# shincling/DL4SS

Measured on AMD Instinct MI355X. Metric: mixtures/sec (8 kHz, 4 s, 2-spk WSJ0-shape) at 1/2/4/8 MI355X, higher is better.
Workload: dtype bf16; 1 GPU; C2: 2-spk pit BiLSTM-4L magnitude mask (EvalVer model), B=32/GPU, N=32000 (T=251,F=129); global_batch=32, seq_len=251, parallelism=dp1, precision=bf16, loss=pit, launch=hip-graph, step=mix+STFT+fwd+loss+bwd+allreduce+Adam

## Files before the change

### dl4ss_amd/csrc/gemm_gl.hip

```cpp
#include "common.h"

#include <algorithm>

namespace {

typedef short bf16x8 __attribute__((ext_vector_type(8)));
typedef short bf16x4 __attribute__((ext_vector_type(4)));
typedef float f32x4 __attribute__((ext_vector_type(4)));
typedef __attribute__((address_space(3))) void lds_void;
typedef __attribute__((address_space(3))) bf16x4 lds_bf16x4;

constexpr int BN = 128, BK = 64;
constexpr int PAN = 128 * BK;

template <int BM_, int STG_, int KT_ = 64>
struct Cfg {
  static constexpr int BM = BM_, STG = STG_, KT = KT_, NT = 2 * BM_, NW = NT / 64;
  static constexpr int PPP = KT_ / 4;
  static constexpr int CPW_A = BM_ * KT_ / 512 / NW, CPW_B = BN * KT_ / 512 / NW;
  static constexpr int IMG_A = BM_ * KT_, IMG_B = BN * KT_, STAGE = IMG_A + IMG_B;
  static constexpr int SMEM = STG_ * STAGE > NW * 32 * 68 * 2 ? STG_ * STAGE : NW * 32 * 68 * 2;
  static constexpr int WPC = NT > 256 ? 1 : SMEM * 2 <= 40 * 1024 ? 4 : SMEM * 2 <= 53 * 1024 ? 3
                             : SMEM * 2 <= 80 * 1024 ? 2 : 1;
  static_assert(CPW_A >= 1 && CPW_B >= 1, "at least one DMA per wave and operand");
// ... 117 lines not shown
#pragma unroll
    for (int kk = 0; kk < KT / 32; ++kk) {
      bf16x8 af[4], bfr[4];
#pragma unroll
      for (int i = 0; i < 4; ++i) af[i] = frag<A_KC, KT>(ia, wm + 16 * i + (lane & 15), kk, lane);
#pragma unroll
      for (int j = 0; j < 4; ++j) bfr[j] = frag<B_KC, KT>(ib, wn + 16 * j + (lane & 15), kk, lane);
#ifndef GGL_NO_MFMA
#pragma unroll
      for (int i = 0; i < 4; ++i)
#pragma unroll
        for (int j = 0; j < 4; ++j) acc[i][j] = __builtin_amdgcn_mfma_f32_16x16x32_bf16(af[i], bfr[j], acc[i][j], 0, 0, 0);
      if constexpr (RS) {
        if (rs) {
#pragma unroll
          for (int i = 0; i < 4; ++i) accr[i] = __builtin_amdgcn_mfma_f32_16x16x32_bf16(af[i], ones, accr[i], 0, 0, 0);
        }
      }
#else
#pragma unroll
      for (int i = 0; i < 4; ++i) asm volatile("" :: "v"(af[i]), "v"(bfr[i]));
#endif
    }
  };
  auto dma = [&](int t) {
    unsigned short* na = smem + (t % STG) * STAGE;
    sa_.issue(na, wave, t, t * KT, kspan);
    sb_.issue(na + IMG_A, wave, t, t * KT, kspan);
  };
  if constexpr (STG == 2) {
    dma(0);
    asm volatile("s_waitcnt vmcnt(0)" ::: "memory");
    __syncthreads();
    for (int kt = 0; kt < nk; ++kt) {
#ifndef GGL_NO_DMA
      if (kt + 1 < nk) dma(kt + 1);
#endif
      compute(smem + (kt & 1) * STAGE);
      asm volatile("s_waitcnt vmcnt(0)" ::: "memory");
      __syncthreads();
    }
  } else {
    constexpr int PW = CF::CPW_A + CF::CPW_B;
#pragma unroll
    for (int t = 0; t < STG - 1; ++t)
      if (t < nk) dma(t);
    for (int kt = 0; kt < nk; ++kt) {
      const int ahead = min(STG - 2, nk - 1 - kt);
      if (ahead >= STG - 2) vm_wait<(STG - 2) * PW>();
      else vm_wait_n<PW, STG - 2>(ahead);
      __builtin_amdgcn_s_barrier();
      if (kt + STG - 1 < nk) dma(kt + STG - 1);
      compute(smem + (kt % STG) * STAGE);
    }
    __syncthreads();
  }

  if constexpr (RS) {
    if (rs && (lane & 15) == 0) {
#pragma unroll
      for (int i = 0; i < 4; ++i)
#pragma unroll
        for (int e = 0; e < 4; ++e) {
          const int row = m0 + wm + 16 * i + 4 * (lane >> 4) + e;
          if (row < M) rsum[row] = beta != 0.0f ? accr[i][e] + beta * rsum[row] : accr[i][e];
        }
    }
  }
  constexpr int SLD = 68;
  float* stage = reinterpret_cast<float*>(smem) + wave * 32 * SLD;
  const int c4 = 4 * (lane & 15);
  const int col = n0 + wn + c4;
  const bool add_bias = !SPLIT && bias != nullptr;
  float4 bv = make_float4(0.f, 0.f, 0.f, 0.f);
  if (add_bias) {
    bv.x = col < N ? bias[col] : 0.f;
    bv.y = col + 1 < N ? bias[col + 1] : 0.f;
    bv.z = col + 2 < N ? bias[col + 2] : 0.f;
    bv.w = col + 3 < N ? bias[col + 3] : 0.f;
  }
  float* out = SPLIT ? slab : C;
  const long long ldo = SPLIT ? N : ldc;
  const bool vec_c = (ldo % 4 == 0) && ((((uintptr_t)out) & 15) == 0) && col + 4 <= N;
#pragma unroll
  for (int h = 0; h < 2; ++h) {
#ifdef GGL_NO_STORE
    if (M > 0) break;
#endif
    __builtin_amdgcn_wave_barrier();
    asm volatile("" ::: "memory");
#pragma unroll
    for (int i2 = 0; i2 < 2; ++i2)
#pragma unroll
      for (int j = 0; j < 4; ++j)
#pragma unroll
        for (int e = 0; e < 4; ++e)
          stage[(16 * i2 + 4 * (lane >> 4) + e) * SLD + 16 * j + (lane & 15)] = acc[2 * h + i2][j][e];
    __builtin_amdgcn_wave_barrier();
    asm volatile("" ::: "memory");
#pragma unroll 4
    for (int rr = 0; rr < 32; rr += 4) {
      const int rl = rr + (lane >> 4);
      const int row = m0 + wm + 32 * h + rl;
      if (row >= M) continue;
      float4 x = *reinterpret_cast<const float4*>(stage + rl * SLD + c4);
      x.x += bv.x; x.y += bv.y; x.z += bv.z; x.w += bv.w;
      if constexpr (EPI == EPI_TANH_BF16) {
        unsigned short* cb = reinterpret_cast<unsigned short*>(C) + (long long)row * ldc + col;
        const float xs[4] = {ftanh_fast(x.x), ftanh_fast(x.y), ftanh_fast(x.z), ftanh_fast(x.w)};
        unsigned short hb[4];
#pragma unroll
        for (int c = 0; c < 4; ++c) {
          hb[c] = (unsigned short)bf16_bits_rne(xs[c]);
        }
        if (col + 4 <= N) {
          *reinterpret_cast<unsigned*>(cb) = hb[0] | ((unsigned)hb[1] << 16);
          *reinterpret_cast<unsigned*>(cb + 2) = hb[2] | ((unsigned)hb[3] << 16);
        } else {
          for (int c = 0; c < 4 && col + c < N; ++c) cb[c] = hb[c];
        }
        continue;
      }
      float* cp = out + (long long)row * ldo + col;
      if (vec_c) {
        if (!SPLIT && beta != 0.0f) {
          const float4 o = *reinterpret_cast<const float4*>(cp);
          x.x += beta * o.x; x.y += beta * o.y; x.z += beta * o.z; x.w += beta * o.w;
        }
        if (EPI == EPI_TANH) { x.x = ftanh_fast(x.x); x.y = ftanh_fast(x.y); x.z = ftanh_fast(x.z); x.w = ftanh_fast(x.w); }
        *reinterpret_cast<float4*>(cp) = x;
      } else {
        const float xs[4] = {x.x, x.y, x.z, x.w};
#pragma unroll
        for (int c = 0; c < 4; ++c) {
          if (col + c >= N) break;
          float y = xs[c];
          if (!SPLIT && beta != 0.0f) y += beta * cp[c];
          if (EPI == EPI_TANH) y = ftanh_fast(y);
          cp[c] = y;
        }
      }
    }
  }
}

template <bool A_KC, bool B_KC, int EPI, bool SPLIT, class CF>
__global__ __launch_bounds__(CF::NT, CF::WPC) void gemm_gl_kernel(
    int M, int N, int K, const unsigned short* __restrict__ A, long long lda, const unsigned short* __restrict__ B,
    long long ldb, float* __restrict__ C, long long ldc, const float* __restrict__ bias, float beta, int k_per_split,
    int grid_m, int grid_n, long long sa, long long sb, long long sc, float* __restrict__ part) {
  constexpr int BM = CF::BM;
  __shared__ __attribute__((aligned(16))) unsigned short smem[CF::SMEM];
  const int ntiles = grid_m * grid_n;
  const int nwg = gridDim.x * gridDim.y * gridDim.z;
  const int L = blockIdx.x + gridDim.x * (blockIdx.y + gridDim.y * blockIdx.z);
  const int xcd = L % 8, q8 = nwg / 8, r8 = nwg % 8;
  const int R = (xcd < r8 ? xcd * (q8 + 1) : r8 * (q8 + 1) + (xcd - r8) * q8) + L / 8;
  const int zsplit = R / (ntiles * (int)gridDim.y);
  const int ymem = (R / ntiles) % (int)gridDim.y;
  const int tile = R % ntiles;
  A += ymem * sa;
  B += ymem * sb;
  C += ymem * sc;
  constexpr int GROUP = 8;
  const int gsize = GROUP * grid_n;
  const int first_m = (tile / gsize) * GROUP;
  const int gm_here = min(grid_m - first_m, GROUP);
  const int tm = first_m + (tile % gsize) % gm_here, tn = (tile % gsize) / gm_here;
  const int m0 = tm * BM, n0 = tn * BN;
  const int kbeg = zsplit * k_per_split;
  const int kend = min(K, kbeg + k_per_split);
  if (kbeg >= kend) return;
  gl_tile<A_KC, B_KC, EPI, SPLIT, CF>(smem, M, N, A, lda, B, ldb, C, ldc, bias, beta, m0, n0, kbeg, kend - kbeg,
                                      SPLIT ? part + ((long long)ymem * gridDim.z + zsplit) * M * N : nullptr);
}

template <int EPI, bool SPLIT>
__device__ __forceinline__ void store4(float4 x, int row, int col, int N, float* C, long long ldc, float* out,
                                       long long ldo, bool vec_c, float beta, const float4& bv) {
  x.x += bv.x; x.y += bv.y; x.z += bv.z; x.w += bv.w;
  if constexpr (EPI == EPI_TANH_BF16) {
    unsigned short* cb = reinterpret_cast<unsigned short*>(C) + (long long)row * ldc + col;
// ... 632 lines not shown
```

### dl4ss_amd/engine.py

```python
import ctypes

import torch

from . import _lib, adam, dp, ops
from .adversarial import AdvStep
from .ops import CELLS, DEFER_BIAS, DGH_PAD8, DOUT_SLABS, WS_ZEROED, pad8
from .params import DiscNet, FlatParams, SepNet, _ngate
from .plan import RETIRED_KNOBS, check_args, step_plan
from .imagequery import ImageQueryStep
from .voiceprint import VoiceprintStep


class SepTrainer:

    def __init__(self, net, batch, k, n_samples, mode="label", precision="fp32", lr=2e-4, sum_weight=0.5,
                 loss_channels=None, betas=(0.9, 0.999), eps=1e-8, process_group=None, rnn_precision=None,
                 adversary=None, adv_weight=1.0, adv_lr=None, disc_adv_update=True, clip_norm=None,
                 adv_clip_norm=None, voiceprint=None, memory=None, voiceprint_lr=None, memory_refresh="reference",
                 splitk_reduce="atomic", image_query=None, image_query_lr=None, optimizer="adam",
                 schedule_decay=0.004, clipnorm=None):
        self.clip_norm, self.adv_clip_norm = check_args(
            net, batch, k, n_samples, mode, precision, rnn_precision, loss_channels, process_group, adversary,
            clip_norm, adv_clip_norm, voiceprint, memory, memory_refresh, splitk_reduce=splitk_reduce,
            inet=image_query, optimizer=optimizer, schedule_decay=schedule_decay, clipnorm=clipnorm)
        self.optimizer, self.schedule_decay = optimizer, float(schedule_decay)
        self.clipnorm = None if clipnorm is None else float(clipnorm)
        self.inet = image_query
        self.vnet, self.memory, self.memory_refresh, self.adversary = voiceprint, memory, memory_refresh, adversary
        self.align = getattr(net, "attention", "dot") == "align"
        vars(self).update(vars(step_plan(net, batch, n_samples, precision, rnn_precision, process_group)))
        self.net, self.B, self.K, self.N = net, batch, k, n_samples
        self.mode, self.precision = mode, precision
        self._sk = 1 if (self.align and not self.fast) else "auto"
        self.splitk_reduce = splitk_reduce
        self._gk = {}
        if splitk_reduce == "fixed":
            self._sk = "auto"
        self.pg = process_group
        self.world = dp.world(process_group) if process_group is not None else 1
        self.T = ops.n_frames(n_samples)
        self.F = net.F
        dev = net.device
        B, K, N, T, F, H = batch, k, n_samples, self.T, net.F, net.H
        NGH = _ngate(net.cell) * H
        BT, FE = B * T, F * net.E
        f32 = dict(device=dev, dtype=torch.float32)
        self._sig = torch.empty(B + B * K, N, **f32)
        self.mix = self._sig[:B]
        self.src = self._sig[B:].view(B, K, N)
        self.stats = torch.empty(32 * B * K, **f32)
        if mode == "crm":
            self.mag_mix = torch.empty(B, T, F, **f32)
            self.Xc_mix = torch.empty(B, T, F, 2, **f32)
            self.Xc_src = torch.empty(B, K, T, F, 2, **f32)
        else:
            self.Xc_mix = None
            self._mag = torch.empty(B + B * K * (2 if adversary is not None else 1), T, F, **f32)
            self.mag_mix = self._mag[:B]
            self.mag_src = self._mag[B:B + B * K].view(B, K, T, F)
        self.out = [torch.empty(B, T, 2 * H, **f32) for _ in range(net.L)]
        self.hprev = [torch.empty(B, T, 2 * H, **f32) for _ in range(net.L)]
        self.act = [torch.empty(B, T, 2, 4 * H, **f32) for _ in range(net.L)]
        self.cs = [torch.empty(B, T, 2, H, **f32) for _ in range(net.L)] if net.cell == "lstm" else None
        self.G = torch.empty(BT, 2 * NGH, **f32)
        self.dGh = torch.empty(BT, 2 * NGH, **f32) if net.cell == "gru" else None
        self.dH = [torch.empty(BT, 2 * H, **f32), torch.empty(BT, 2 * H, **f32)]
        self.V = torch.empty(BT, FE, **f32)
        if splitk_reduce == "fixed":
            shapes = [(FE, 2 * H, BT), (BT, 2 * H, FE), (NGH, H, BT), (BT, 2 * H, 2 * NGH)]
            shapes += [(2 * NGH, F if l == 0 else 2 * H, BT) for l in range(net.L)]
            nb = max(ops.gemm_fixed_ws_bytes(*s, "auto") for s in shapes)
            self.fixed_ws = torch.empty(max(nb, 4) // 4, **f32)
            self.cs_part = ops.vp_colsum_part(BT, max(FE, 2 * NGH), dev)
            self._gk = dict(reduce="fixed", ws=self.fixed_ws)
        W = net.W
        self.q = torch.empty(B, K, W, **f32)
        self.mean = torch.empty(B, 2 * H, **f32)
        self.dq = torch.empty(B, K, W, **f32)
        self.dh_bcast = torch.empty(B, 2 * H, **f32)
        self.nblk = _lib.query("dl4ss_attn_align_nblk", T * F) if self.align else _lib.query("dl4ss_attn_nblk", T, F)
        self.part_loss = torch.empty(B, self.nblk, K * K + 1, **f32)
        self.part_dq = torch.empty(B, self.nblk, K, W, **f32)
        if self.align:
            self.part_att = torch.empty(_lib.query("dl4ss_attn_align_part_floats", B, K, self.nblk), **f32)
        self.perm = torch.empty(B, K, device=dev, dtype=torch.int32)
        self.loss = torch.zeros(3, **f32)
        self.eval_out = torch.zeros(3, **f32)
        ws = _lib.query("dl4ss_birnn_workspace_bytes", CELLS[net.cell], B, H)
        if ws < 0:
            raise RuntimeError("unsupported BiRNN configuration")
        self.ws_bytes = ws
        self.rnn_ws = torch.empty((ws + 7) // 8, device=dev, dtype=torch.int64)
        w8 = (ws + 255) // 256 * 32
        self.rnn_ws_all = torch.zeros(2, net.L * w8, device=dev, dtype=torch.int64)
        self._w8 = w8
        self.status = torch.zeros(2, device=dev, dtype=torch.int32)
        okw = dict(kind=optimizer, schedule_decay=schedule_decay, clipnorm=self.clipnorm)
        query_net = voiceprint if voiceprint is not None else image_query
        if self.clipnorm is not None and query_net is not None:
            n0 = ops.grad_sumsq_parts(net.flat.numel())
            joint = torch.zeros(n0 + ops.grad_sumsq_parts(query_net.flat.numel()), dtype=torch.float64, device=dev)
            okw.update(parts=(joint, 0))
        self.opt = adam.GuardedAdam(net.flat, self.status, self.loss, lr, betas, eps, clip_norm=self.clip_norm, **okw)
        if okw.get("parts"):
            okw.update(parts=(joint, n0))
        self.m, self.v = self.opt.m, self.opt.v
        if self.opt.clip is not None:
            self.grad_norm, self._nonfinite = self.opt.grad_norm, self.opt.nonfinite
        nch = loss_channels if loss_channels else K
        self.s1 = 1.0 / (B * nch * T * F)
        self.s2 = 0.0 if (mode == "crm" or loss_channels) else sum_weight / (B * T * F)
        self.spk = torch.empty(B, K, device=dev, dtype=torch.int32)
        self._works = []
        self._in_chain = False
        self._side_stream = self._side_gemm = self._fork_ev = None
        self._wb_ver = None
        self.adv = self.adv_opt = self.vp = None
        if adversary is not None:
            self.adv = AdvStep(adversary, B, K, self._mag, precision, self.status, self.loss,
                               lr if adv_lr is None else adv_lr, betas, eps, adv_weight, disc_adv_update,
                               self.adv_clip_norm)
            a = self.adv
            self.adv_opt, self.adv_m, self.adv_v, self.adv_weight = a.opt, a.opt.m, a.opt.v, a.adv_weight
            self.adv_loss, self.adv_scores, self.gext, self._dmaps, self._dy = a.adv_loss, a.scores, a.gext, a.maps, a.y
            if self.adv_clip_norm is not None:
                self.adv_grad_norm = self.adv_opt.grad_norm
        if voiceprint is not None:
            self.vp = VoiceprintStep(voiceprint, memory, memory_refresh, self.mag_src, self.spk, self.q, self.dq,
                                     self.status, self.loss, lr if voiceprint_lr is None else voiceprint_lr, betas, eps,
                                     wgrad_split="auto" if splitk_reduce == "fixed" else 1, opt_kw=okw)
            self.vp_enc, self.vp_opt = self.vp.enc, self.vp.opt
        self.images = None
        if image_query is not None:
            self.images = torch.zeros(B, K, image_query.h, image_query.w, **f32)
            self.vp = ImageQueryStep(image_query, memory, memory_refresh, self.images, self.spk, self.q, self.dq,
                                     self.status, self.loss, lr if image_query_lr is None else image_query_lr, betas,
                                     eps, opt_kw=okw)
            self.vp_enc, self.vp_opt = self.vp.enc, self.vp.opt
        if not self.fast:
            return
        bf = dict(device=dev, dtype=torch.bfloat16)
        self.xb0 = torch.zeros(BT, pad8(F), **bf)
        self.outb = [torch.empty(BT, pad8(2 * H), **bf) for _ in range(net.L)]
        self.hprevb = [torch.empty(BT, 2 * pad8(H), **bf) for _ in range(net.L)]
        self.dGb_l = [torch.empty(BT, 2 * NGH, **bf) for _ in range(net.L)]
        self.ngh_p8 = pad8(NGH)
        self.dGhb_l = [torch.empty(BT, 2 * self.ngh_p8, **bf) for _ in range(net.L)] if net.cell == "gru" else None
        self._dw_group = None
        self.dPreb = torch.zeros(BT, pad8(FE), **bf)
        gl_need = max(_lib.query("dl4ss_gemm_bf16_gl_ws_bytes", BT, 2 * H, FE, max(1, self.dh_split), 1),
                      _lib.query("dl4ss_gemm_bf16_gl_ws_bytes", BT, 2 * H, 2 * NGH, 1, 1),
                      _lib.query("dl4ss_gemm_bf16_gl_ws_bytes", FE, 2 * H, BT, 2, 1),
                      _lib.query("dl4ss_gemm_bf16_gl_ws_bytes", 2 * NGH, 2 * H, BT, 4, 1),
                      _lib.query("dl4ss_gemm_bf16_gl_ws_bytes", NGH, H, BT, 8, 2))
        self.gl_ws = torch.empty(max(gl_need, 1), device=dev, dtype=torch.uint8)
        if self.dh_slabs > 1:
            self.dh_ws = torch.empty(self.dh_slabs * BT * 2 * H * 4, device=dev, dtype=torch.uint8)
        pb = _lib.query("dl4ss_colsum_bf16_part_bytes", BT, FE)
        self.colsum_part = torch.empty(max(1, pb // 4), device=dev, dtype=torch.float32)
        self.Vb = None if self.split else torch.empty(BT, FE, **bf)
        self.wb_ih = [torch.empty(2 * NGH, pad8(F if l == 0 else 2 * H), **bf) for l in range(net.L)]
        self.wb_lin = torch.empty(FE, pad8(2 * H), **bf)
        if self.split:
            self.seg = [pad8(F if l == 0 else 2 * H) for l in range(net.L)]
            self.xs0 = torch.empty(BT, 3 * self.seg[0], **bf)
            self.xs = torch.empty(BT, 3 * pad8(2 * H), **bf)
            self.ws_ih = [torch.empty(2 * NGH, 3 * self.seg[l], **bf) for l in range(net.L)]
            self.ws_lin = torch.empty(FE, 3 * pad8(2 * H), **bf)
        if net.cell == "lstm":
            self.hprev = [None] * net.L

    lr, adv_lr, vp_lr = (adam.delegate(o, "lr") for o in ("opt", "adv_opt", "vp_opt"))
    step_count = adam.delegate("opt", "step_count")
    skipped_nonfinite = adam.delegate("opt", "skipped_nonfinite")
    adv_step_count = adam.delegate("adv_opt", "step_count")
    adv_skipped_nonfinite = adam.delegate("adv_opt", "skipped_nonfinite", default=0)

    def features(self, raw, gains, lengths=None):
        ops.mix_sources(raw, gains, out_src=self.src, out_mix=self.mix, stats_ws=self.stats, lengths=lengths)
        self._stfts()

    def _stfts(self):
        B, K, N = self.B, self.K, self.N
        xb = dict(out_bf16=self.xb0, n_bf16=B) if self.fast else {}
        if self.mode == "crm":
            ops.stft(self.mix, complex_out=True, mag_out=True, out_c=self.Xc_mix, out_mag=self.mag_mix, **xb)
            ops.stft(self.src.view(B * K, N), complex_out=True, mag_out=False, out_c=self.Xc_src.view(B * K, self.T,
                                                                                                     self.F, 2))
        else:
            ops.stft(self._sig, complex_out=False, mag_out=True, out_mag=self._mag, **xb)
        self._xb0_fresh = self.fast

    def _to_bf16_rows(self, x, out):
        _lib.call("dl4ss_f32_to_bf16_2d", _lib.ptr(x, True), x.stride(0), x.shape[0], x.shape[1], _lib.ptr(out),
                  out.stride(0), _lib.stream_ptr())

    def params_changed(self):
        self.net.params_changed()
        self._wb_ver = None

    def _wb_key(self):
        return (self.net.generation, self.net.flat._version)

    def _wb_stale(self):
        return self._wb_ver is None or self._wb_ver != self._wb_key()

    def _weights_to_bf16(self, force=False):
        net = self.net
        if not hasattr(self, "_cvt_args"):
            pairs = [(net.cat_view("weight_ih", l), self.wb_ih[l]) for l in range(net.L)]
            pairs.append((net.view("mix.Linear.weight"), self.wb_lin))
            n = len(pairs)
            P = ctypes.c_void_p
            self._cvt_args = (n, (P * n)(*[x.data_ptr() for x, _ in pairs]),
                              (ctypes.c_longlong * n)(*[x.stride(0) for x, _ in pairs]),
                              (ctypes.c_int * n)(*[x.shape[0] for x, _ in pairs]),
                              (ctypes.c_int * n)(*[x.shape[1] for x, _ in pairs]),
                              (P * n)(*[y.data_ptr() for _, y in pairs]),
                              (ctypes.c_longlong * n)(*[y.stride(0) for _, y in pairs]))
            base = net.flat.data_ptr()
            assert all(x.is_contiguous() for x, _ in pairs)
            self._shadow = (n, (ctypes.c_longlong * n)(*[(x.data_ptr() - base) // 4 for x, _ in pairs]),
                            self._cvt_args[3], self._cvt_args[4], self._cvt_args[5], self._cvt_args[6])
        if not force and self._shadow_on and not self._wb_stale():
            return
        _lib.call("dl4ss_f32_to_bf16_2d_multi", *self._cvt_args, _lib.stream_ptr())
        self._wb_ver = self._wb_key()

    def _forward_prepare(self, x):
        net = self.net
        if self._ws_fill:
            self.rnn_ws_all.zero_()
        self._weights_to_bf16()
        if self.split:
            for l in range(net.L):
                pat, nseg = (ops.W_SPLIT2, 2) if (l >= 1 and self.split_x2) else (ops.W_SPLIT, 3)
                ops.hilo(net.cat_view("weight_ih", l), self.ws_ih[l], self.seg[l], pat, nseg)
            ops.hilo(net.view("mix.Linear.weight"), self.ws_lin, pad8(2 * net.H), ops.W_SPLIT)
        if not self._xb0_ok:
            self._to_bf16_rows(x, self.xb0)
        if self.split:
            ops.hilo(x, self.xs0, self.seg[0], ops.A_SPLIT)

    def _split_input(self, l):
        H, w = self.net.H, pad8(2 * self.net.H)
# ... 560 lines not shown
```

### dl4ss_amd/ops.py

```python
import torch

from . import _lib

_C = _lib.CONSTANTS
STFT_COMPLEX, STFT_MAG, STFT_LOGMAG, STFT_CONJ = (_C["DL4SS_STFT_" + n] for n in ("COMPLEX", "MAG", "LOGMAG", "CONJ"))
N_FFT, HOP = 256, 128
F_BINS = N_FFT // 2 + 1


def n_frames(n_samples):
    return 1 + n_samples // HOP


def _f32c(t, name):
    if not (t.is_cuda and t.dtype == torch.float32 and t.is_contiguous()):
        raise RuntimeError(f"{name}: expected a contiguous float32 CUDA tensor")
    return t


def stft(x, complex_out=True, mag_out=True, log=False, conj=False, out_c=None, out_mag=None, out_bf16=None,
         n_bf16=0):
    _f32c(x, "stft")
    N = x.shape[-1]
    lead = x.shape[:-1]
# ... 432 lines not shown

def disc_forward(prec, maps, params, ys, logit, score):
    w1, b1, w2, b2, w3, b3, wf, bf = (_lib.ptr(p) for p in params)
    (N, T, F), (y1, y2, y3), st = maps.shape, ys, _lib.stream_ptr()
    _lib.call("dl4ss_disc_conv1_fwd", prec, _lib.ptr(maps), w1, b1, N, T, F, _lib.ptr(y1), st)
    for x, y, w, b in ((y1, y2, w2, b2), (y2, y3, w3, b3)):
        _lib.call("dl4ss_disc_conv64_fwd", prec, _lib.ptr(x), w, b, N, x.shape[1], x.shape[2], _lib.ptr(y), st)
    _lib.call("dl4ss_disc_head_fwd", prec=prec, y3=_lib.ptr(y3), wf=wf, bf=bf, N=N, H3=y3.shape[1], W3=y3.shape[2],
              z=_lib.ptr(logit), score=_lib.ptr(score), stream=st)


def disc_backward(prec, maps, weights, ys, dys, score, dscore, target, loss, dz, grads, dx, ws, ws_bytes):
    w1, w2, w3, wf = (_lib.ptr(w) for w in weights)
    dw1, db1, dw2, db2, dw3, db3, dwf, dbf = (_lib.ptr(g) for g in grads)
    (N, T, F), (y1, y2, y3), (d1, d2, d3), ws, st = maps.shape, ys, dys, _lib.ptr(ws), _lib.stream_ptr()
    _lib.call("dl4ss_disc_head_bwd", prec=prec, y3=_lib.ptr(y3), wf=wf, score=_lib.ptr(score), dscore=_lib.ptr(dscore),
              target=float(target), N=N, H3=y3.shape[1], W3=y3.shape[2], loss=_lib.ptr(loss), dz=_lib.ptr(dz), dwf=dwf,
              dbf=dbf, dy3=_lib.ptr(d3), stream=st)
    for x, y, dy, w, dx_, dw, db in ((y2, y3, d3, w3, d2, dw3, db3), (y1, y2, d2, w2, d1, dw2, db2)):
        _lib.call("dl4ss_disc_conv64_bwd", prec=prec, x=_lib.ptr(x), y=_lib.ptr(y), dy=_lib.ptr(dy), w=w, N=N,
                  Hin=x.shape[1], Win=x.shape[2], dx=_lib.ptr(dx_), dw=dw, db=db, ws=ws, ws_bytes=ws_bytes, stream=st)
    _lib.call("dl4ss_disc_conv1_bwd", prec=prec, x=_lib.ptr(maps), y1=_lib.ptr(y1), dy1=_lib.ptr(d1), w=w1, N=N, T=T,
              F=F, dx=_lib.ptr(dx), dw=dw1, db=db1, ws=ws, ws_bytes=ws_bytes, stream=st)


CELLS = {"lstm": _C["DL4SS_CELL_LSTM"], "gru": _C["DL4SS_CELL_GRU"]}
WS_ZEROED = _C["DL4SS_RNN_WS_ZEROED"]
DGH_PAD8 = _C["DL4SS_RNN_DGH_PAD8"]
DEFER_BIAS = _C["DL4SS_RNN_DEFER_BIAS"]
HARD_GATES = _C["DL4SS_RNN_HARD_GATES"]
GATES = ("logistic", "hard")


def gate_flags(gates, cell="lstm", precision="fp32"):
    if gates not in GATES:
        raise ValueError(f"gates {gates!r}: expected one of {GATES}")
    if gates == "logistic":
        return 0
    if cell != "lstm":
        raise ValueError(f"gates='hard' is Keras 1's LSTM cell: cell {cell!r} has no hard-gates form")
    if PREC[precision] != 0:
        raise ValueError("gates='hard' (Keras 1's LSTM cell) needs the fp32 recurrence: the packed bf16 recurrence "
                         f"has no hard-gates form (the recurrence resolves to {precision!r}; use precision='fp32', "
                         "or precision='bf16' with rnn_precision='fp32')")
    return HARD_GATES


def DOUT_SLABS(n):
    return ((n - 1) & 3) << 12


def birnn_fwd(cell, B, T, H, *, G, w_hh, b_hh, act, ws, ws_bytes, status, out=None, hprev=None, cs=None,
              out_bf16=None, hprev_bf16=None, h_mean=None, precision="fp32", flags=0):
    p = _lib.ptr
    _lib.call("dl4ss_birnn_fwd_mean", CELLS[cell], PREC[precision] | flags, B, T, H, p(G), p(w_hh), p(b_hh), p(out),
              p(hprev), p(act), p(cs), p(out_bf16), p(hprev_bf16), p(h_mean), p(ws), ws_bytes, p(status),
              _lib.stream_ptr())


def birnn_fwd_xw(cell, B, T, H, *, x, w_ih, b_ih, w_hh, b_hh, act, ws, ws_bytes, status, out=None, hprev=None,
                 cs=None, out_bf16=None, hprev_bf16=None, h_mean=None, ws_zeroed=True):
    p = _lib.ptr
    _lib.call("dl4ss_birnn_fwd_xw_ex", CELLS[cell], B, T, H, p(x, True), x.shape[1], x.stride(0), p(w_ih, True),
              w_ih.stride(0), p(b_ih), p(w_hh), p(b_hh), p(out), p(hprev), p(act), p(cs), p(out_bf16), p(hprev_bf16),
              p(h_mean), p(ws), ws_bytes, p(status), _lib.stream_ptr(), int(ws_zeroed))


def birnn_bwd(cell, B, T, H, *, w_hh, act, ws, ws_bytes, status, dOut=None, dOut_bcast=None, cs=None, hprev=None,
              dG=None, dGh=None, dG_bf16=None, dGh_bf16=None, db_ih=None, db_hh=None, precision="fp32", flags=0):
    p = _lib.ptr
    _lib.call("dl4ss_birnn_bwd_ex", CELLS[cell], PREC[precision] | flags, B, T, H, p(dOut), p(dOut_bcast), p(w_hh),
              p(act), p(cs), p(hprev), p(dG), p(dGh), p(dG_bf16), p(dGh_bf16), p(db_ih), p(db_hh), p(ws), ws_bytes,
              p(status), _lib.stream_ptr())


A_SPLIT, W_SPLIT = 0b010, 0b100
A_SPLIT2, W_SPLIT2 = 0b00, 0b10


def pad8(n):
    return (n + 7) // 8 * 8


def hilo(x, y, segw, pattern, nseg=3):
    _lib.call("dl4ss_f32_to_bf16_hilo", x=_lib.ptr(x, True), ldx=x.stride(0), rows=x.shape[0], cols=x.shape[1],
              y=_lib.ptr(y), ldy=y.stride(0), segw=segw, nseg=nseg, pattern=pattern, stream=_lib.stream_ptr())


def birnn_plan(cell, B, H, precision="bf16", max_wg=0):
    import ctypes

    info = (ctypes.c_int * 5)()
    rc = _lib.lib().dl4ss_birnn_plan_info(CELLS[cell], int(B), int(H),
                                          1 if precision == "bf16" else 0, int(max_wg), info)
    if rc != 0:
        return None
    return dict(zip(("BC", "NG", "J", "nchunk", "grid"), list(info)))


VP_RULES = {"nonzero": 0, "gt": 1}


def _i32c(t, name, numel):
    if not (t.is_cuda and t.dtype == torch.int32 and t.is_contiguous() and t.numel() == numel):
        raise RuntimeError(f"{name}: expected a contiguous int32 CUDA tensor of {numel} elements")
    return t


def vp_compact(x, rule="nonzero", thr=None, lengths=None, xc=None, len_out=None, idx=None):
    _f32c(x, "vp_compact")
    if x.dim() != 3:
        raise RuntimeError("vp_compact: expected (n, T, F)")
    if rule not in VP_RULES:
        raise ValueError(f"vp_compact: rule {rule!r}, expected one of {sorted(VP_RULES)}")
    if rule == "gt" and thr is None and lengths is None:
        raise ValueError("vp_compact: rule 'gt' needs thr")
    n, T, F = x.shape
    if lengths is not None:
        _i32c(lengths, "vp_compact(lengths)", n)
    i32 = dict(device=x.device, dtype=torch.int32)
    xc = torch.empty_like(x) if xc is None else _f32c(xc, "vp_compact(xc)")
    len_out = torch.empty(n, **i32) if len_out is None else _i32c(len_out, "vp_compact(len)", n)
    idx = torch.empty(n, T, **i32) if idx is None else _i32c(idx, "vp_compact(idx)", n * T)
    if xc.numel() != x.numel():
        raise RuntimeError("vp_compact: xc must have x's size")
    _lib.call("dl4ss_vp_compact", x=_lib.ptr(x), n=n, T=T, F=F, rule=VP_RULES[rule],
              thr=float(0.0 if thr is None else thr), len_in=_lib.ptr(lengths), xc=_lib.ptr(xc), len=_lib.ptr(len_out),
              idx=_lib.ptr(idx), stream=_lib.stream_ptr())
    return xc, len_out, idx


def vp_shift(src, dst, lengths, c0, c1, direction, other=0):
    _f32c(src, "vp_shift(src)")
    _f32c(dst, "vp_shift(dst)")
    if src.dim() != 3 or src.shape != dst.shape:
        raise RuntimeError("vp_shift: src and dst must be (n, T, ld) of one shape")
    n, T, ld = src.shape
    _i32c(lengths, "vp_shift(lengths)", n)
    _lib.call("dl4ss_vp_shift", src=_lib.ptr(src), dst=_lib.ptr(dst), n=n, T=T, ld=ld, c0=int(c0), c1=int(c1),
              len=_lib.ptr(lengths), dir=int(direction), other=int(other), stream=_lib.stream_ptr())
    return dst


def vp_mean_fwd(out, lengths, vec=None):
    _f32c(out, "vp_mean_fwd")
    n, T, D = out.shape
    _i32c(lengths, "vp_mean_fwd(lengths)", n)
    vec = torch.empty(n, D, device=out.device, dtype=torch.float32) if vec is None else _f32c(vec, "vp_mean_fwd(vec)")
    if D % 2 or vec.numel() != n * D:
        raise RuntimeError("vp_mean_fwd: out (n, T, 2H), vec (n, 2H)")
    _lib.call("dl4ss_vp_mean_fwd", _lib.ptr(out), n, T, D // 2, _lib.ptr(lengths), _lib.ptr(vec), _lib.stream_ptr())
    return vec


def vp_mean_bwd(dvec, lengths, dout):
    _f32c(dvec, "vp_mean_bwd")
    _f32c(dout, "vp_mean_bwd(dout)")
    n, T, D = dout.shape
    _i32c(lengths, "vp_mean_bwd(lengths)", n)
    if D % 2 or dvec.numel() != n * D:
        raise RuntimeError("vp_mean_bwd: dvec (n, 2H), dout (n, T, 2H)")
    _lib.call("dl4ss_vp_mean_bwd", _lib.ptr(dvec), n, T, D // 2, _lib.ptr(lengths), _lib.ptr(dout), _lib.stream_ptr())
    return dout


def vp_colsum_part(M, C, device):
# ... 122 lines not shown
```

### dl4ss_amd/plan.py

```python
import os
import types

import torch

from . import _lib, ops
from .imagequery import ImageQueryNet
from .params import DiscNet, _ngate
from .voiceprint import SpeakerMemory, VoiceprintNet


def _same_device(net, other):
    return (other.device.type, other.device.index or 0) == (net.device.type, net.device.index or 0)


def check_optimizer(optimizer, schedule_decay, clip_norm, clipnorm):
    if optimizer not in ("adam", "nadam"):
        raise ValueError(f"optimizer {optimizer!r}: expected 'adam' or 'nadam'")
    if not float(schedule_decay) >= 0.0:
        raise ValueError(f"schedule_decay must not be negative, got {schedule_decay}")
    if clipnorm is None:
        return None
    if clip_norm is not None:
        raise ValueError("clip_norm (torch.nn.utils.clip_grad_norm_'s rule) and clipnorm (Keras's rule) are given "
                         "together: choose one")
# ... 71 lines not shown
        if net.E != vnet.E:
            raise ValueError(f"voiceprint: the encoder's vectors have {vnet.E} elements, the net's queries {net.E}")
        if memory.E != vnet.E:
            raise ValueError(f"memory: rows of {memory.E} elements, the encoder's vectors have {vnet.E}")
        if net.F != vnet.F:
            raise ValueError(f"voiceprint: the encoder reads {vnet.F} bins, the step's magnitudes have {net.F}")
        if precision != "fp32":
            raise ValueError(f"voiceprint: precision {precision!r} is unsupported, the voiceprint path is fp32")
        if loss_channels:
            raise ValueError("voiceprint: loss_channels is unsupported")
        if adversary is not None:
            raise ValueError("voiceprint: an adversary is unsupported")
        if process_group is not None:
            raise ValueError("voiceprint: no data-parallel voiceprint step (process_group; the encoder's gradient "
                             "and the memory are not all-reduced)")
        if clip_norm is not None:
            raise ValueError("voiceprint: clip_norm is unsupported (one global norm over the two flat gradients "
                             "needs a kernel change)")
        if memory_refresh not in ("reference", "reuse"):
            raise ValueError(f"memory_refresh {memory_refresh!r}: expected 'reference' or 'reuse'")
        if batch * k > 1024:
            raise ValueError(f"voiceprint: {batch * k} sources per step, the memory kernels take at most 1024")
        for what, other in (("voiceprint", vnet), ("memory", memory)):
            if not _same_device(net, other):
                raise ValueError(f"{what}: lives on another device than the net")
    clip_norm = None if clip_norm is None else ops.check_clip_norm(clip_norm)
    adv_clip_norm = None if adv_clip_norm is None else ops.check_clip_norm(adv_clip_norm, "adv_clip_norm")
    if adv_clip_norm is not None and adversary is None:
        raise ValueError("adv_clip_norm needs an adversary")
    if (mode == "crm") != net.crm:
        raise ValueError("cRM mode needs a cRM net (query width 2E) and vice versa")
    check_hard_gates(net, resolve_rnn_precision(precision, rnn_precision))
    align = getattr(net, "attention", "dot") == "align"
    if adversary is not None:
        T = ops.n_frames(n_samples)
        if not isinstance(adversary, DiscNet):
            raise ValueError("adversary: expected an engine.DiscNet")
        if mode == "crm":
            raise ValueError("adversary: the adversarial term is built for the magnitude modes, not 'crm'")
        if loss_channels:
            raise ValueError("adversary: loss_channels is unsupported with an adversary")
        if align:
            raise ValueError("adversary: attention='align' is unsupported with an adversary")
        if process_group is not None:
            raise ValueError("adversary: no data-parallel adversarial step (the Discriminator's gradients are "
                             "not all-reduced)")
        if T < 15:
            raise ValueError(f"adversary: {T} frames, the Discriminator needs maps of at least 15 x 15")
        if (adversary.T, adversary.F) != (T, net.F):
            raise ValueError(f"adversary: a DiscNet for ({adversary.T}, {adversary.F}) maps, this trainer's "
                             f"are ({T}, {net.F})")
        if not _same_device(net, adversary):
            raise ValueError("adversary: the DiscNet lives on another device than the net")
    if align:
        if mode == "crm":
            raise ValueError("attention='align' supports the modes 'label' and 'pit', not 'crm'")
        if loss_channels:
            raise ValueError("attention='align' does not support loss_channels")
        fast = precision in ("bf16s", "bf16s2") or (precision == "bf16" and (rnn_precision or precision) == "bf16")
        if fast and net.cell != "lstm":
            raise ValueError(f"attention='align' on the bf16 / bf16s fast paths is built for cell 'lstm', not "
                             f"{net.cell!r} (precision={precision!r}, rnn_precision={rnn_precision!r}); use "
                             "precision='fp32'")
        if net.E != 50:
            raise ValueError("attention='align' is built for embedding size 50")
    return clip_norm, adv_clip_norm


RETIRED_KNOBS = ("DL4SS_DX_SPLIT", "DL4SS_DEFER_BIAS", "DL4SS_SIDE_LATE", "DL4SS_DW_SPLITS", "DL4SS_DW_CFG") + \
    _lib.RETIRED_ENV


def resolve_rnn_precision(precision, rnn_precision=None):
    if precision in ("bf16s", "bf16s2") and rnn_precision in (None, precision):
        return "bf16"
    return rnn_precision or precision


def check_hard_gates(net, rnn_precision):
    gates = getattr(net, "gates", "logistic")
    return ops.gate_flags(gates, net.cell, rnn_precision) if gates != "logistic" else 0


def step_plan(net, batch, n_samples, precision, rnn_precision=None, process_group=None):
    env = os.environ
    for name in RETIRED_KNOBS:
        if name in env:
            raise ValueError(f"{name} is retired, its default is the only path (DESIGN.md section 11): unset it")
    p = types.SimpleNamespace()
    B, T, F, H, L = batch, ops.n_frames(n_samples), net.F, net.H, net.L
    BT, FE, NGH = B * T, F * net.E, _ngate(net.cell) * H
    p.split = precision in ("bf16s", "bf16s2")
    p.split_x2 = precision == "bf16s2"
    p.rnn_precision = resolve_rnn_precision(precision, rnn_precision)
    p.rnn_flags = check_hard_gates(net, p.rnn_precision)
    if p.split and p.rnn_precision != "bf16":
        raise ValueError(f"precision '{precision}' runs the bf16 recurrence (rnn_precision bf16)")
    p.fast = precision in ("bf16", "bf16s", "bf16s2") and p.rnn_precision == "bf16"
    p.grouped = L <= 5
    p._ws_fill = T < 4 or env.get("DL4SS_WS_FILL", "0") == "1"
    p.dh_split = int(env.get("DL4SS_DH_SPLIT", "3"))
    xw = env.get("DL4SS_RNN_XW", "1")
    if xw not in ("0", "1", "l0"):
        raise ValueError(f"DL4SS_RNN_XW={xw}: expected 0, 1 or l0")
    p.xw = p.fast and xw != "0" and not p.split
    p.xw_kmax = 160 if xw == "l0" else 640
    p.xw_split0 = p.split and xw != "0"
    nb = env.get("DL4SS_DP_BUCKETS", "2")
    if nb not in ("0", "1", "2", "3"):
        raise ValueError(f"DL4SS_DP_BUCKETS={nb}: expected 0, 1 (alias of 2), 2 or 3")
    p.buckets = process_group is not None and p.fast and p.grouped and nb != "0"
    p.dp_layer = L // 2 if (p.buckets and nb == "3" and L >= 2) else None
    p.zero_free = p.fast and p.grouped and env.get("DL4SS_GRAD_ZERO", "0") != "1"
    p._gbeta = 0.0 if p.zero_free else 1.0
    p._shadow_on = p.fast and env.get("DL4SS_ADAM_SHADOW", "1") != "0"
    cuda = net.device.type == "cuda"
    rnn = ops.birnn_plan(net.cell, B, H) if (p.fast and cuda) else None
    p.side = None
    side = env.get("DL4SS_SIDE_DWLIN", "")
    if p.fast and p.grouped and side != "0" and cuda:
        if side and side != "1":
            v = [int(x) for x in side.split(",")]
            p.side = (v[0], v[1], v[2], bool(v[3]) if len(v) > 3 else True)
        else:
            cus = torch.cuda.get_device_properties(net.device).multi_processor_count
            free = cus - (rnn["grid"] if rnn else 1 << 30)
            flops = 2.0 * FE * (2 * H) * BT
            if free >= 8 and (flops / (free * 2.75e12) < L * T * 1.75e-6 * 0.85 or side == "1"):
                p.side = (free, 2, 1, False)
    p.dh_slabs = 1
    if p.fast and env.get("DL4SS_DH_SLABS", "1") != "0" and rnn is not None and rnn["BC"] == 4:
        nsl = _lib.query("dl4ss_gemm_bf16_gl_ws_bytes", BT, 2 * H, FE, max(1, p.dh_split), 1) // (BT * 2 * H * 4)
        p.dh_slabs = 3 if nsl == 3 else 1

    def tiles(m, n):
        return ((m + 127) // 128) * ((n + 127) // 128)

    wg1 = 2 * tiles(FE, 2 * H) + sum(tiles(2 * NGH, F if l == 0 else 2 * H) for l in range(L)) + \
        4 * 2 * L * tiles(NGH, H)
    p.dw_splits = (2, 1 if wg1 >= 3 * 512 else 2, 4)
    return p
```

Before: 9626 mixtures/s.

## Pad dPreb and wb_lin rows to 64-element pitch; widen tanh-bf16 epilogue stores

Adds a row-pitch plan that, by default, pads the rows of the dPreb gradient buffer and the bf16 linear weight to a multiple of 64 elements, so each row starts on a 128-byte line. The GEMM tanh-bf16 epilogue also gains a wide path in which each lane writes 8 bf16 values as one 16-byte store instead of two 4-byte stores. Both changes aim to cut partial-line and misaligned global memory traffic. The cost is extra padding memory, and any consumer that assumed the old pad8 pitch must read the stride correctly.

```diff
diff --git a/dl4ss_amd/csrc/gemm_gl.hip b/dl4ss_amd/csrc/gemm_gl.hip
--- a/dl4ss_amd/csrc/gemm_gl.hip
+++ b/dl4ss_amd/csrc/gemm_gl.hip
@@ -223,6 +223,17 @@
   float* out = SPLIT ? slab : C;
   const long long ldo = SPLIT ? N : ldc;
   const bool vec_c = (ldo % 4 == 0) && ((((uintptr_t)out) & 15) == 0) && col + 4 <= N;
+  bool wide = false;
+  const int c8 = 8 * (lane & 7);
+  const int col8 = n0 + wn + c8;
+  float bw[8] = {0.f, 0.f, 0.f, 0.f, 0.f, 0.f, 0.f, 0.f};
+  if constexpr (EPI == EPI_TANH_BF16) {
+    wide = (ldc % 8 == 0) && ((((uintptr_t)C) & 15) == 0);
+    if (wide && add_bias) {
+#pragma unroll
+      for (int c = 0; c < 8; ++c) bw[c] = col8 + c < N ? bias[col8 + c] : 0.f;
+    }
+  }
 #pragma unroll
   for (int h = 0; h < 2; ++h) {
 #ifdef GGL_NO_STORE
@@ -239,6 +250,35 @@
           stage[(16 * i2 + 4 * (lane >> 4) + e) * SLD + 16 * j + (lane & 15)] = acc[2 * h + i2][j][e];
     __builtin_amdgcn_wave_barrier();
     asm volatile("" ::: "memory");
+    if constexpr (EPI == EPI_TANH_BF16) {
+      if (wide) {
+#pragma unroll 2
+        for (int rr = 0; rr < 32; rr += 8) {
+          const int rl = rr + (lane >> 3);
+          const int row = m0 + wm + 32 * h + rl;
+          if (row >= M || col8 >= N) continue;
+          const float4 x0 = *reinterpret_cast<const float4*>(stage + rl * SLD + c8);
+          const float4 x1 = *reinterpret_cast<const float4*>(stage + rl * SLD + c8 + 4);
+          const float xs[8] = {x0.x + bw[0], x0.y + bw[1], x0.z + bw[2], x0.w + bw[3],
+                               x1.x + bw[4], x1.y + bw[5], x1.z + bw[6], x1.w + bw[7]};
+          unsigned hb[8];
+#pragma unroll
+          for (int c = 0; c < 8; ++c) hb[c] = bf16_bits_rne(ftanh_fast(xs[c])) & 0xFFFFu;
+          unsigned short* cb = reinterpret_cast<unsigned short*>(C) + (long long)row * ldc + col8;
+          if (col8 + 8 <= N) {
+            *reinterpret_cast<uint4*>(cb) = make_uint4(hb[0] | (hb[1] << 16), hb[2] | (hb[3] << 16),
+                                                       hb[4] | (hb[5] << 16), hb[6] | (hb[7] << 16));
+          } else {
+#pragma unroll
+            for (int c = 0; c < 8; c += 2) {
+              if (col8 + c + 2 <= N) *reinterpret_cast<unsigned*>(cb + c) = hb[c] | (hb[c + 1] << 16);
+              else if (col8 + c < N) cb[c] = (unsigned short)hb[c];
+            }
+          }
+        }
+        continue;
+      }
+    }
 #pragma unroll 4
     for (int rr = 0; rr < 32; rr += 4) {
       const int rl = rr + (lane >> 4);
diff --git a/dl4ss_amd/engine.py b/dl4ss_amd/engine.py
--- a/dl4ss_amd/engine.py
+++ b/dl4ss_amd/engine.py
@@ -18,7 +18,7 @@
                  adversary=None, adv_weight=1.0, adv_lr=None, disc_adv_update=True, clip_norm=None,
                  adv_clip_norm=None, voiceprint=None, memory=None, voiceprint_lr=None, memory_refresh="reference",
                  splitk_reduce="atomic", image_query=None, image_query_lr=None, optimizer="adam",
-                 schedule_decay=0.004, clipnorm=None):
+                 schedule_decay=0.004, clipnorm=None, row_pitch=None):
         self.clip_norm, self.adv_clip_norm = check_args(
             net, batch, k, n_samples, mode, precision, rnn_precision, loss_channels, process_group, adversary,
             clip_norm, adv_clip_norm, voiceprint, memory, memory_refresh, splitk_reduce=splitk_reduce,
@@ -28,7 +28,7 @@
         self.inet = image_query
         self.vnet, self.memory, self.memory_refresh, self.adversary = voiceprint, memory, memory_refresh, adversary
         self.align = getattr(net, "attention", "dot") == "align"
-        vars(self).update(vars(step_plan(net, batch, n_samples, precision, rnn_precision, process_group)))
+        vars(self).update(vars(step_plan(net, batch, n_samples, precision, rnn_precision, process_group, row_pitch)))
         self.net, self.B, self.K, self.N = net, batch, k, n_samples
         self.mode, self.precision = mode, precision
         self._sk = 1 if (self.align and not self.fast) else "auto"
@@ -140,6 +140,7 @@
         if not self.fast:
             return
         bf = dict(device=dev, dtype=torch.bfloat16)
+        pitch = self.pitch
         self.xb0 = torch.zeros(BT, pad8(F), **bf)
         self.outb = [torch.empty(BT, pad8(2 * H), **bf) for _ in range(net.L)]
         self.hprevb = [torch.empty(BT, 2 * pad8(H), **bf) for _ in range(net.L)]
@@ -147,7 +148,7 @@
         self.ngh_p8 = pad8(NGH)
         self.dGhb_l = [torch.empty(BT, 2 * self.ngh_p8, **bf) for _ in range(net.L)] if net.cell == "gru" else None
         self._dw_group = None
-        self.dPreb = torch.zeros(BT, pad8(FE), **bf)
+        self.dPreb = torch.zeros(BT, pitch["dPreb"], **bf)
         gl_need = max(_lib.query("dl4ss_gemm_bf16_gl_ws_bytes", BT, 2 * H, FE, max(1, self.dh_split), 1),
                       _lib.query("dl4ss_gemm_bf16_gl_ws_bytes", BT, 2 * H, 2 * NGH, 1, 1),
                       _lib.query("dl4ss_gemm_bf16_gl_ws_bytes", FE, 2 * H, BT, 2, 1),
@@ -160,7 +161,8 @@
         self.colsum_part = torch.empty(max(1, pb // 4), device=dev, dtype=torch.float32)
         self.Vb = None if self.split else torch.empty(BT, FE, **bf)
         self.wb_ih = [torch.empty(2 * NGH, pad8(F if l == 0 else 2 * H), **bf) for l in range(net.L)]
-        self.wb_lin = torch.empty(FE, pad8(2 * H), **bf)
+        self.wb_lin = torch.empty(FE, pad8(2 * H), **bf) if pitch["wb_lin"] == pad8(2 * H) else \
+            torch.zeros(FE, pitch["wb_lin"], **bf)
         if self.split:
             self.seg = [pad8(F if l == 0 else 2 * H) for l in range(net.L)]
             self.xs0 = torch.empty(BT, 3 * self.seg[0], **bf)
diff --git a/dl4ss_amd/ops.py b/dl4ss_amd/ops.py
--- a/dl4ss_amd/ops.py
+++ b/dl4ss_amd/ops.py
@@ -538,6 +538,10 @@
     return (n + 7) // 8 * 8
 
 
+def pad_line(n):
+    return (n + 63) // 64 * 64
+
+
 def hilo(x, y, segw, pattern, nseg=3):
     _lib.call("dl4ss_f32_to_bf16_hilo", x=_lib.ptr(x, True), ldx=x.stride(0), rows=x.shape[0], cols=x.shape[1],
               y=_lib.ptr(y), ldy=y.stride(0), segw=segw, nseg=nseg, pattern=pattern, stream=_lib.stream_ptr())
diff --git a/dl4ss_amd/plan.py b/dl4ss_amd/plan.py
--- a/dl4ss_amd/plan.py
+++ b/dl4ss_amd/plan.py
@@ -177,7 +177,23 @@
     return ops.gate_flags(gates, net.cell, rnn_precision) if gates != "logistic" else 0
 
 
-def step_plan(net, batch, n_samples, precision, rnn_precision=None, process_group=None):
+ROW_PITCHES = ("line", "legacy")
+
+
+def row_pitches(net, row_pitch):
+    if row_pitch not in ROW_PITCHES:
+        raise ValueError(f"row_pitch={row_pitch!r}: expected one of {ROW_PITCHES}")
+    F, H, FE, NGH = net.F, net.H, net.F * net.E, _ngate(net.cell) * net.H
+    p = dict(xb0=ops.pad8(F), outb=ops.pad8(2 * H), hprevb=2 * ops.pad8(H), dGb=2 * NGH, dPreb=ops.pad8(FE), Vb=FE,
+             wb_ih0=ops.pad8(F), wb_ih=ops.pad8(2 * H), wb_lin=ops.pad8(2 * H))
+    if row_pitch == "line":
+        p["wb_lin"] = ops.pad_line(2 * H)
+        if getattr(net, "attention", "dot") != "align":
+            p["dPreb"] = ops.pad_line(FE)
+    return p
+
+
+def step_plan(net, batch, n_samples, precision, rnn_precision=None, process_group=None, row_pitch=None):
     env = os.environ
     for name in RETIRED_KNOBS:
         if name in env:
@@ -209,6 +225,8 @@
     p.zero_free = p.fast and p.grouped and env.get("DL4SS_GRAD_ZERO", "0") != "1"
     p._gbeta = 0.0 if p.zero_free else 1.0
     p._shadow_on = p.fast and env.get("DL4SS_ADAM_SHADOW", "1") != "0"
+    p.row_pitch = row_pitch if row_pitch is not None else env.get("DL4SS_ROW_PITCH", "line")
+    p.pitch = row_pitches(net, p.row_pitch)
     cuda = net.device.type == "cuda"
     rnn = ops.birnn_plan(net.cell, B, H) if (p.fast and cuda) else None
     p.side = None
```

Result: no change. 9614 mixtures/s (-0.1%).
